# ChampiB/CBO_with_OOP

Measured on AMD Instinct MI355X. Metric: candidate-intervention acquisitions/sec (16k grid, d=3), higher is better.
Workload: dtype f64

## Files before the change

cbo_with_oop_amd/csrc/kernels_trsm.hip:

```cpp
#include <cstdlib>
#include <type_traits>

#include "cbo_internal.h"

namespace cbo {

#define MFMA_F64(a, b, c) __builtin_amdgcn_mfma_f64_16x16x4f64((a), (b), (c), 0, 0, 0)

#define SCHED_DS(n) __builtin_amdgcn_sched_group_barrier(0x100, (n), 0)
#define SCHED_MFMA(n) __builtin_amdgcn_sched_group_barrier(0x008, (n), 0)
#define SCHED_VMEM(n) __builtin_amdgcn_sched_group_barrier(0x010, (n), 0)

constexpr int kRB = 128;
constexpr int kT = kRB / 16;
constexpr int kLdsLd = kRB + 16;
constexpr int kNBuf = 3;
template <int KB>
struct StageGeom {
    static constexpr int kA = KB * kLdsLd;
    static constexpr int kB = 4 * KB * 16;
    static constexpr int kRA = KB / 4;
    static constexpr int kParts = KB / 8;
    static constexpr int kDma = 3 * kParts;
    static constexpr int kKS = KB / 4;
// ... 950 lines not shown
                    }
                    x = MFMA_F64(iv[2], -acc[m][2], x);
                    x2 = MFMA_F64(iv[3], -acc[m][3], x2);
                    __builtin_amdgcn_sched_barrier(0);
                    x += x2;
                    asm volatile("" : "+v"(x));
#pragma unroll
                    for (int r = 0; r < 4; ++r) xreg[(kq + 4 * r) * 16 + lc] = x[r];
                    PSTAMP(3);
                    asm volatile("s_waitcnt lgkmcnt(0)" ::: "memory");
                    __builtin_amdgcn_s_barrier();
                    __builtin_amdgcn_s_setprio(0);
                    PSTAMP(1);
#pragma unroll
                    for (int t = m + 1; t < kT; ++t)
#pragma unroll
                        for (int kk = 0; kk < 4; ++kk) uf[t][kk] = abase0[(4 * kk) * kPLd + 16 * t];
                    if (SWEEP) {
#pragma unroll
                        for (int r = 0; r < 4; ++r) zr[r] = zl[zpar + 16 * m + kq + 4 * r];
                    }
#pragma unroll
                    for (int kk = 0; kk < 4; ++kk) {
                        if (m + 1 < kT) acc[m + 1] = MFMA_F64(uf[m + 1][kk], x[kk], acc[m + 1]);
                        if (m + 2 < kT) acc[m + 2] = MFMA_F64(uf[m + 2][kk], x[kk], acc[m + 2]);
                        __builtin_amdgcn_sched_barrier(0);
                        if (kk == 0) { issue_one(ahead, bnext, 0); issue_one(ahead, bnext, 1); }
                        else if (kk == 1) { issue_one(ahead, bnext, 2); issue_one(ahead, bnext, 3); }
                        else if (kk == 2) issue_one(ahead, bnext, 4);
                        else advance(ahead);
                        __builtin_amdgcn_sched_barrier(0);
                    }
#pragma unroll
                    for (int r = 0; r < 4; ++r) {
                        asm volatile("global_store_dwordx2 %0, %1, %2" ::"v"(vq_off), "v"(x[r]), "s"(V + colw + (int64_t)(i0 + 16 * m + 4 * r) * ldv) : "memory");
                        if (SWEEP) {
                            qacc = fma(x[r], x[r], qacc);
                            macc = fma(x[r], zr[r], macc);
                        }
                    }
                    if (SWEEP) asm volatile("" : "+v"(qacc), "+v"(macc));
#pragma unroll
                    for (int kk = 0; kk < 4; ++kk)
#pragma unroll
                        for (int t = m + 3; t < kT; ++t) acc[t] = MFMA_F64(uf[t][kk], x[kk], acc[t]);
                    a1 += 4;
                    if (SWEEP && m == kPD0 - 1) {
                        hand[0] = qacc;
                        hand[1] = macc;
                        qacc = 0.0;
                        macc = 0.0;
                    }
                    PSTAMP(2); PSTAMP_NEXT(); buf = (buf == 2) ? 0 : buf + 1;
                }
#pragma unroll
                for (int m = 0; m < kPD1; ++m) {
                    wait_top();
                    const int bnext = (buf >= 1) ? buf - 1 : 2;
                    issue_stage(ahead, bnext);
                    advance(ahead);
                    if (m < 2) {
#pragma unroll
                        for (int sl = (m == 0 ? 0 : kL0); sl < (m == 0 ? kL0 : kAhead); ++sl) {
                            request_one(i0, sl);
                            __builtin_amdgcn_s_sleep(2);
                        }
                        a1 += m == 0 ? kL0 : kL1;
                    }
                    PSTAMP(2); PSTAMP_NEXT(); buf = (buf == 2) ? 0 : buf + 1;
                }
            } else {
#pragma unroll
                for (int m = 0; m < kPD0; ++m) {
                    wait_top();
                    const int bnext = (buf >= 1) ? buf - 1 : 2;
                    const double *abase0 = lds + buf * kPA + kq * kPLd + lc;
                    double *xreg = ldsB + buf * kPBd + cw * 256;
                    double uf[kT][4], xb[4];
#pragma unroll
                    for (int t = 0; t < kT; ++t) {
                        if (m > 0 || !P0) acc[t] = MFMA_F64(af[1][t], bf[1], acc[t]);
#pragma unroll
                        for (int kk = 0; kk < 4; ++kk) uf[t][kk] = abase0[(4 * kk) * kPLd + kRB + 16 * t];
                    }
                    PSTAMP(3);
                    asm volatile("s_waitcnt lgkmcnt(0)" ::: "memory");
                    __builtin_amdgcn_s_barrier();
                    PSTAMP(1);
#pragma unroll
                    for (int kk = 0; kk < 4; ++kk) xb[kk] = xreg[(4 * kk + kq) * 16 + lc];
#pragma unroll
                    for (int kk = 0; kk < (m + 1 < kPD0 ? 3 : 4); ++kk)
#pragma unroll
                        for (int t = 0; t < kT; ++t) {
                            acc[t] = MFMA_F64(uf[t][kk], xb[kk], acc[t]);
                            const int slot = kk * kT + t;
                            if (slot < kPDma) issue_one(ahead, bnext, slot);
                            else if (slot == kPDma) step(ahead);
                            else if (slot == kPDma + 1) locate_a(ahead);
                            else if (slot == kPDma + 2) locate_b(ahead);
                            else if (slot == kPDma + 3) locate_c(ahead);
                            __builtin_amdgcn_sched_barrier(0);
                        }
                    if (m + 1 < kPD0) {
#pragma unroll
                        for (int t = 0; t < kT; ++t) af[1][t] = uf[t][3];
                        bf[1] = xb[3];
                    }
                    PSTAMP(2); PSTAMP_NEXT(); buf = (buf == 2) ? 0 : buf + 1;
                }
#pragma unroll
                for (int m = 0; m < kPD1; ++m) {
                    wait_top();
                    const int bnext = (buf >= 1) ? buf - 1 : 2;
                    constexpr int kTl = kT;
                    const int s = 2 * m;
                    const double *ab = lds + buf * kPA + kq * kPLd + lc;
                    const double *ivb = ldsB + buf * kPBd + kq * 16 + lc;
                    double iv[2][4], uf[2][kTl][4], zr[2][4];
                    if (SWEEP && m == 0) {
                        qacc = hand[0];
                        macc = hand[1];
                    }
#pragma unroll
                    for (int kk = 0; kk < 4; ++kk) iv[0][kk] = ivb[(4 * kk) * 16];
                    d4 x = {0.0, 0.0, 0.0, 0.0}, x2 = {0.0, 0.0, 0.0, 0.0};
                    x = MFMA_F64(iv[0][0], -acc[s][0], x);
                    x2 = MFMA_F64(iv[0][1], -acc[s][1], x2);
                    x = MFMA_F64(iv[0][2], -acc[s][2], x);
                    x2 = MFMA_F64(iv[0][3], -acc[s][3], x2);
                    __builtin_amdgcn_sched_barrier(0);
#pragma unroll
                    for (int kk = 0; kk < 4; ++kk) iv[1][kk] = ivb[256 + (4 * kk) * 16];
#pragma unroll
                    for (int t = s + 1; t < kT; ++t)
#pragma unroll
                        for (int kk = 0; kk < 4; ++kk) uf[0][t][kk] = ab[(4 * kk) * kPLd + 16 * t];
                    if (SWEEP) {
#pragma unroll
                        for (int hh = 0; hh < 2; ++hh)
#pragma unroll
                            for (int r = 0; r < 4; ++r) zr[hh][r] = zl[zpar + kRB + 16 * (s + hh) + kq + 4 * r];
                    }
                    __builtin_amdgcn_sched_barrier(0);
                    x += x2;
                    asm volatile("" : "+v"(x));
                    PSTAMP(1);
                    auto emit = [&](int hh, const d4 &xx) __attribute__((always_inline)) {
#pragma unroll
                        for (int r = 0; r < 4; ++r) {
                            asm volatile("global_store_dwordx2 %0, %1, %2" ::"v"(vq_off), "v"(xx[r]), "s"(V + colw + (int64_t)(i0 + kRB + 16 * (s + hh) + 4 * r) * ldv) : "memory");
                            if (SWEEP) {
                                qacc = fma(xx[r], xx[r], qacc);
                                macc = fma(xx[r], zr[hh][r], macc);
                            }
                        }
                        if (SWEEP) asm volatile("" : "+v"(qacc), "+v"(macc));
                    };
#pragma unroll
                    for (int kk = 0; kk < 4; ++kk) {
                        acc[s + 1] = MFMA_F64(uf[0][s + 1][kk], x[kk], acc[s + 1]);
                        if (s + 2 < kT) acc[s + 2] = MFMA_F64(uf[0][s + 2][kk], x[kk], acc[s + 2]);
                        __builtin_amdgcn_sched_barrier(0);
                        if (kk == 0) { issue_one(ahead, bnext, 0); issue_one(ahead, bnext, 1); }
                        else if (kk == 1) { issue_one(ahead, bnext, 2); issue_one(ahead, bnext, 3); }
                        else if (kk == 2) issue_one(ahead, bnext, 4);
                        else advance(ahead);
                        __builtin_amdgcn_sched_barrier(0);
                    }
                    emit(0, x);
                    const d4 na = -acc[s + 1];
                    d4 y1 = {0.0, 0.0, 0.0, 0.0}, y2 = {0.0, 0.0, 0.0, 0.0};
#pragma unroll
                    for (int kk = 0; kk < 4; ++kk) {
                        if (kk & 1) y2 = MFMA_F64(iv[1][kk], na[kk], y2);
                        else y1 = MFMA_F64(iv[1][kk], na[kk], y1);
#pragma unroll
                        for (int t = s + 3; t < kT; ++t) {
                            acc[t] = MFMA_F64(uf[0][t][kk], x[kk], acc[t]);
                            if (SWEEP && m == 1 && kk == 0 && t == s + 3) request_one(i0, kT * 4);
                        }
                    }
#pragma unroll
                    for (int t = s + 2; t < kT; ++t)
#pragma unroll
                        for (int kk = 0; kk < 4; ++kk) uf[1][t][kk] = ab[(4 * kk) * kPLd + kRB + 16 * t];
                    const d4 y = y1 + y2;
                    emit(1, y);
#pragma unroll
                    for (int kk = 0; kk < 4; ++kk)
#pragma unroll
                        for (int t = s + 2; t < kT; ++t) {
                            acc[t] = MFMA_F64(uf[1][t][kk], y[kk], acc[t]);
                            const int idx = kk * (kT - s - 2) + (t - s - 2);
                            if (m < 2 && idx < 16) request_one(i0, 16 * m + idx);
                        }
                    a1 += 8 + (m == 0 ? kL0 : m == 1 ? kL1 : 0);
                    if (SWEEP && m == kPD1 - 1) {
                        qacc += __shfl_xor(qacc, 16);
                        qacc += __shfl_xor(qacc, 32);
                        macc += __shfl_xor(macc, 16);
                        macc += __shfl_xor(macc, 32);
                        qtot += qacc;
                        mtot += macc;
                        qacc = 0.0;
                        macc = 0.0;
                    }
                    PSTAMP(2); PSTAMP_NEXT(); buf = (buf == 2) ? 0 : buf + 1;
                }
            }
        };
        diag_phase(0, std::true_type{});
        for (int i0 = kPB; i0 < n; i0 += kPB) {
            const int nst = i0 / kPKB;
            regular_stage(i0, std::true_type{});
            for (int j = 1; j < nst; ++j) regular_stage(i0, std::false_type{});
            diag_phase(i0, std::false_type{});
        }
        asm volatile("s_waitcnt vmcnt(0)" ::: "memory");
        __builtin_amdgcn_s_barrier();

        if (SWEEP && H == 1 && kq == 0) {
            q_out[colw + lc] = qtot;
            mu_out[colw + lc] = mtot;
        }
    };
    if (h == 0) run(std::integral_constant<int, 0>{});
    else run(std::integral_constant<int, 1>{});
#undef PSTAMP
#undef PSTAMP_NEXT
}

constexpr int kAccMoves = kT * 4;

template <int KB>
__global__ __launch_bounds__(256) void trsm_update_kernel(const double *__restrict__ U, int64_t ldu,
                                                          const double *V, int64_t ldv, double *C, int64_t ldc, int k0,
                                                          int klen, int i0_begin, int i0_end, int chunk_rows,
                                                          int upper_only, const int *__restrict__ skip_if)
{
    if (skip_if && __builtin_nontemporal_load(skip_if) != 0) return;
    using G = StageGeom<KB>;
    constexpr int kA = G::kA, kB = G::kB, kRA = G::kRA, kParts = G::kParts, kDma = G::kDma, kKS = G::kKS;
    __shared__ __align__(16) double lds[kNBuf * (kA + kB)];

    const int tid = threadIdx.x;
#ifdef CBO_DIAG_KNOBS
    const unsigned long long upd_t0 = __builtin_amdgcn_s_memtime();
    const unsigned long long upd_r0 = __builtin_amdgcn_s_memrealtime();
    const int upd_id = (int)(blockIdx.y * gridDim.x + blockIdx.x);
    const bool upd_probe = tid == 0 && blockIdx.x == 7 && blockIdx.y == gridDim.y / 2;
    int upd_k = 0;
#define UPD_STAMP() do { if (upd_probe && upd_k < 128) g_upd_stage[upd_k++] = __builtin_amdgcn_s_memtime(); } while (0)
#else
#define UPD_STAMP() do { } while (0)
#endif
    const int lane = tid & 63;
    const int wave = __builtin_amdgcn_readfirstlane(tid >> 6);
    const int lc = lane & 15, kq = lane >> 4;
    const int64_t colw = (int64_t)blockIdx.x * kStrip + wave * 16;
    const int ib = i0_begin + (int)blockIdx.y * chunk_rows;
    const int ie = (ib + chunk_rows < i0_end) ? ib + chunk_rows : i0_end;
    if (ib >= ie) return;
    if (upper_only && (int)blockIdx.x * kStrip + kStrip <= ib) return;
    const int nst = klen / KB;
    double *Cc = C + colw + lc;
    double *ldsB = lds + kNBuf * kA;
    const unsigned lds_byte0 = lds_byte_address(lds);
    const double *ug = U + (int64_t)(k0 + wave * kRA) * ldu + lane * 2;
    const double *vg = V + (int64_t)(k0 + (lane >> 3)) * ldv + colw + 2 * (lane & 7);
    const int64_t b_stride = 8 * ldv;

    int ci0 = ib, cj = 0;
    const double *a_src, *b_src;
    auto locate = [&]() __attribute__((always_inline)) {
        const bool past = ci0 >= ie;
        const int ai0 = past ? ie - kRB : ci0;
        const int aj = past ? nst - 1 : cj;
        a_src = ug + (int64_t)(KB * aj) * ldu + ai0;
        b_src = vg + (int64_t)(KB * aj) * ldv;
    };
    auto advance = [&]() __attribute__((always_inline)) {
        const int wrap = (cj + 1 == nst) ? 1 : 0;
        ci0 += kRB * wrap;
        cj = (cj + 1) * (1 - wrap);
        locate();
    };
    auto issue_one = [&](int buf, int part, int q) __attribute__((always_inline)) {
        if (q < 2) {
            const unsigned la = __builtin_amdgcn_readfirstlane(lds_byte0 + 8u * (unsigned)(buf * kA + (wave * kRA) * kLdsLd));
            const int p = 2 * part + q;
            glds16(a_src + (int64_t)p * ldu, la + 8u * (unsigned)(p * kLdsLd));
        } else {
            const unsigned lb = __builtin_amdgcn_readfirstlane(
                lds_byte0 + 8u * (unsigned)(kNBuf * kA + buf * kB + wave * (KB * 16)));
            glds16(b_src + part * b_stride, lb + 8u * (unsigned)(part * 128));
        }
    };
    auto issue_part = [&](int buf, int part) __attribute__((always_inline)) {
#pragma unroll
        for (int q = 0; q < 3; ++q) issue_one(buf, part, q);
    };

    d4 acc[kT], accn[kT];
#pragma unroll
    for (int t = 0; t < kT; ++t)
#pragma unroll
        for (int r = 0; r < 4; ++r) acc[t][r] = -Cc[(int64_t)(ib + 16 * t + kq + 4 * r) * ldc];

    UPD_STAMP();
    locate();
#pragma unroll
    for (int part = 0; part < kParts; ++part) issue_part(0, part);
    advance();
#pragma unroll
    for (int part = 0; part < kParts; ++part) issue_part(1, part);
    advance();
    UPD_STAMP();

    int buf = 0;
    int boundary = 0;
    for (int i0 = ib; i0 < ie; i0 += kRB) {
        double af[2][kT], bf[2];
        bool deferred = false;
        for (int j = 0; j < nst; ++j) {
            asm volatile("s_waitcnt lgkmcnt(0)" ::: "memory");
            if (boundary) asm volatile("s_waitcnt vmcnt(%0)" ::"n"(kDma + kAccMoves) : "memory");
            else asm volatile("s_waitcnt vmcnt(%0)" ::"n"(kDma) : "memory");
            __builtin_amdgcn_s_barrier();
            UPD_STAMP();
            boundary = (boundary > 0) ? boundary - 1 : 0;
            if (j == 0 && i0 + kRB < ie) {
#pragma unroll
                for (int t = 0; t < kT; ++t)
#pragma unroll
                    for (int r = 0; r < 4; ++r) accn[t][r] = -Cc[(int64_t)(i0 + kRB + 16 * t + kq + 4 * r) * ldc];
                asm volatile("" ::: "memory");
            }
            __builtin_amdgcn_sched_barrier(0);
            const int bnext = (buf >= 1) ? buf - 1 : 2;
            const double *abase = lds + buf * kA + kq * kLdsLd + lc;
            const double *bbase = ldsB + buf * kB + wave * (KB * 16) + kq * 16 + lc;
#pragma unroll
            for (int t = 0; t < kT; ++t) {
                if (deferred) acc[t] = MFMA_F64(af[1][t], bf[1], acc[t]);
                if (t < kT / 2) {
                    af[0][2 * t] = abase[32 * t];
                    af[0][2 * t + 1] = abase[32 * t + 16];
                } else if (t == kT / 2) {
                    bf[0] = bbase[0];
                }
                __builtin_amdgcn_sched_barrier(0);
            }
#pragma unroll
            for (int jj = 0; jj < kKS - 1; ++jj) {
                const double *an = abase + 4 * (jj + 1) * kLdsLd;
#pragma unroll
                for (int t = 0; t < kT; ++t) {
                    acc[t] = MFMA_F64(af[jj & 1][t], bf[jj & 1], acc[t]);
                    if (t < kT / 2) {
                        af[(jj + 1) & 1][2 * t] = an[32 * t];
                        af[(jj + 1) & 1][2 * t + 1] = an[32 * t + 16];
                    } else if (t == kT / 2) {
                        bf[(jj + 1) & 1] = bbase[4 * (jj + 1) * 16];
                    } else if (jj < kParts) {
                        issue_one(bnext, jj, t - (kT / 2 + 1));
                    } else if (jj == kParts && t == kT / 2 + 1) {
                        advance();
                    }
                    __builtin_amdgcn_sched_barrier(0);
                }
            }
            deferred = true;
            buf = (buf == 2) ? 0 : buf + 1;
        }
#pragma unroll
        for (int t = 0; t < kT; ++t) acc[t] = MFMA_F64(af[1][t], bf[1], acc[t]);
        UPD_STAMP();
#pragma unroll
        for (int t = 0; t < kT; ++t)
#pragma unroll
            for (int r = 0; r < 4; ++r) Cc[(int64_t)(i0 + 16 * t + kq + 4 * r) * ldc] = -acc[t][r];
        asm volatile("" ::: "memory");
        UPD_STAMP();
#pragma unroll
        for (int t = 0; t < kT; ++t) acc[t] = accn[t];
        boundary = 2;
    }
    asm volatile("s_waitcnt vmcnt(0)" ::: "memory");
    __builtin_amdgcn_s_barrier();
#ifdef CBO_DIAG_KNOBS
    UPD_STAMP();
    if (tid == 0 && upd_id < 65536) {
        unsigned hw, xcc;
        asm volatile("s_getreg_b32 %0, hwreg(HW_REG_HW_ID)" : "=s"(hw));
        asm volatile("s_getreg_b32 %0, hwreg(HW_REG_XCC_ID)" : "=s"(xcc));
        g_upd_wg[5 * upd_id] = upd_t0;
        g_upd_wg[5 * upd_id + 1] = __builtin_amdgcn_s_memtime();
        g_upd_wg[5 * upd_id + 2] = (unsigned long long)hw | ((unsigned long long)xcc << 32);
        g_upd_wg[5 * upd_id + 3] = upd_r0;
        g_upd_wg[5 * upd_id + 4] = __builtin_amdgcn_s_memrealtime();
    }
#endif
#undef UPD_STAMP
}

void launch_trsm_strips(hipStream_t s, const double *U, int64_t ldu, const double *invDt, double *V, int64_t ldv,
                        int64_t n, int64_t m_pad, const double *z, double *q, double *mu, bool accumulate,
                        bool half_lds)
{
    if (n <= 0 || m_pad <= 0) return;
    const dim3 grid((unsigned)(m_pad / kStrip));
    const int acc = accumulate ? 1 : 0;
    if (half_lds) {
        if (q != nullptr)
            hipLaunchKernelGGL((trsm_strip_kernel<true, 16>), grid, dim3(256), 0, s, U, ldu, invDt, V, ldv, (int)n, z, q, mu, acc);
        else
            hipLaunchKernelGGL((trsm_strip_kernel<false, 16>), grid, dim3(256), 0, s, U, ldu, invDt, V, ldv, (int)n, z, q, mu, 0);
        return;
    }
    static const bool pairs = [] {
        const char *e = getenv("CBO_HIP_STRIP_FORM");
        return !(e && atoi(e) == 8);
    }();
    if (pairs && n >= kPB && n % kPB == 0) {
#ifdef CBO_DIAG_KNOBS
        static const int pair_mask = [] {
            const char *e = getenv("CBO_HIP_STRIP_MASK");
            return e ? atoi(e) : 0;
        }();
        const int acc = (accumulate ? 1 : 0) | (pair_mask << 8);
#endif
        if (q != nullptr)
            hipLaunchKernelGGL((trsm_pair_kernel<true>), grid, dim3(512), 0, s, U, ldu, invDt, V, ldv, (int)n, z, q, mu, acc);
        else
            hipLaunchKernelGGL((trsm_pair_kernel<false>), grid, dim3(512), 0, s, U, ldu, invDt, V, ldv, (int)n, z, q, mu, 0);
        return;
    }
    if (q != nullptr)
        hipLaunchKernelGGL((trsm_strip8_kernel<true>), grid, dim3(512), 0, s, U, ldu, invDt, V, ldv, (int)n, z, q, mu, acc);
    else
        hipLaunchKernelGGL((trsm_strip8_kernel<false>), grid, dim3(512), 0, s, U, ldu, invDt, V, ldv, (int)n, z, q, mu, 0);
}

void launch_trsm_update(hipStream_t s, const double *U, int64_t ldu, double *V, int64_t ldv, int k0, int klen,
                        int i0_begin, int i0_end, int64_t m_pad, int chunk_blocks, bool half_lds)
{
    launch_gemm_update(s, U, ldu, V, ldv, V, ldv, k0, klen, i0_begin, i0_end, m_pad, chunk_blocks, half_lds, false, nullptr);
}

void launch_gemm_update(hipStream_t s, const double *U, int64_t ldu, const double *V, int64_t ldv, double *C,
                        int64_t ldc, int k0, int klen, int i0_begin, int i0_end, int64_t m_pad, int chunk_blocks,
                        bool half_lds, bool upper_only, const int *skip_if)
{
    if (i0_begin >= i0_end || m_pad <= 0 || klen <= 0) return;
    const int chunk_rows = chunk_blocks * kRB;
    const unsigned chunks = (unsigned)((i0_end - i0_begin + chunk_rows - 1) / chunk_rows);
    const dim3 grid((unsigned)(m_pad / kStrip), chunks);
    const int up = upper_only ? 1 : 0;
    if (!half_lds)
        hipLaunchKernelGGL(trsm_update_kernel<32>, grid, dim3(256), 0, s, U, ldu, V, ldv, C, ldc, k0, klen, i0_begin,
                           i0_end, chunk_rows, up, skip_if);
    else
        hipLaunchKernelGGL(trsm_update_kernel<16>, grid, dim3(256), 0, s, U, ldu, V, ldv, C, ldc, k0, klen, i0_begin,
                           i0_end, chunk_rows, up, skip_if);
}

__global__ void mfma_selftest_kernel(const double *A, const double *B, double *C)
{
    const int l = threadIdx.x;
    d4 acc = {0.0, 0.0, 0.0, 0.0};
    for (int k0 = 0; k0 < 16; k0 += 4)
        acc = MFMA_F64(A[(l & 15) * 16 + k0 + (l >> 4)], B[(k0 + (l >> 4)) * 16 + (l & 15)], acc);
    d4 acc2 = {0.0, 0.0, 0.0, 0.0};
    for (int kk = 0; kk < 4; ++kk) acc2 = MFMA_F64(A[(l & 15) * 16 + 4 * kk + (l >> 4)], acc[kk], acc2);
    for (int r = 0; r < 4; ++r) {
        C[((l >> 4) + 4 * r) * 16 + (l & 15)] = acc[r];
        C[256 + ((l >> 4) + 4 * r) * 16 + (l & 15)] = acc2[r];
    }
}

int run_mfma_selftest(hipStream_t s, double *max_err)
{
    double hA[256], hB[256], hC[512], ref[256], ref2[256];
    for (int i = 0; i < 16; ++i)
        for (int j = 0; j < 16; ++j) {
            hA[i * 16 + j] = (double)((i * 7 + j * 3) % 11 - 5);
            hB[i * 16 + j] = (double)((i * 5 + j * 13 + 1) % 17 - 8);
        }
    for (int i = 0; i < 16; ++i)
        for (int j = 0; j < 16; ++j) {
            double acc = 0.0;
            for (int k = 0; k < 16; ++k) acc += hA[i * 16 + k] * hB[k * 16 + j];
            ref[i * 16 + j] = acc;
        }
    for (int i = 0; i < 16; ++i)
        for (int j = 0; j < 16; ++j) {
            double acc = 0.0;
            for (int k = 0; k < 16; ++k) acc += hA[i * 16 + k] * ref[k * 16 + j];
            ref2[i * 16 + j] = acc;
        }
    double *dA = nullptr, *dB = nullptr, *dC = nullptr;
    if (hipMalloc(&dA, sizeof(hA)) != hipSuccess || hipMalloc(&dB, sizeof(hB)) != hipSuccess ||
        hipMalloc(&dC, sizeof(hC)) != hipSuccess)
        return -1;
    hipMemcpyAsync(dA, hA, sizeof(hA), hipMemcpyHostToDevice, s);
    hipMemcpyAsync(dB, hB, sizeof(hB), hipMemcpyHostToDevice, s);
    hipLaunchKernelGGL(mfma_selftest_kernel, dim3(1), dim3(64), 0, s, dA, dB, dC);
    hipMemcpyAsync(hC, dC, sizeof(hC), hipMemcpyDeviceToHost, s);
    const hipError_t e = hipStreamSynchronize(s);
    hipFree(dA); hipFree(dB); hipFree(dC);
    if (e != hipSuccess) return -1;
    double m = 0.0;
    for (int i = 0; i < 256; ++i) {
        const double e1 = fabs(hC[i] - ref[i]), e2 = fabs(hC[256 + i] - ref2[i]);
        if (e1 > m) m = e1;
        if (e2 > m) m = e2;
    }
    *max_err = m;
    return 0;
}

}
```

Before: 3.053 million.

## Prefetch next C strip via inline-asm loads spread across stages with tracked vmcnt

Replaces the compiler-generated prefetch of the next accumulator strip, which was issued in one burst at stage 0, with inline-asm global loads. These are split into two batches of 16, issued after the MFMA loops of stages 0 and 1. A young-load counter selects the matching s_waitcnt vmcnt so the LDS DMA waits do not also wait on the C prefetch. The negation of the loaded C values moves until after the initial DMA issue or the strip boundary. This is meant to hide C load latency behind MFMA work and avoid stalls at strip boundaries. In exchange it relies on fragile manual vmcnt accounting (including kAccMoves) and carries a correctness risk if the counts mismatch.

```diff
diff --git a/cbo_with_oop_amd/csrc/kernels_trsm.hip b/cbo_with_oop_amd/csrc/kernels_trsm.hip
--- a/cbo_with_oop_amd/csrc/kernels_trsm.hip
+++ b/cbo_with_oop_amd/csrc/kernels_trsm.hip
@@ -1276,13 +1276,13 @@
         for (int q = 0; q < 3; ++q) issue_one(buf, part, q);
     };
 
-    d4 acc[kT], accn[kT];
+    d4 acc[kT];
+    double accn[kT][4];
 #pragma unroll
     for (int t = 0; t < kT; ++t)
 #pragma unroll
-        for (int r = 0; r < 4; ++r) acc[t][r] = -Cc[(int64_t)(ib + 16 * t + kq + 4 * r) * ldc];
-
-    UPD_STAMP();
+        for (int r = 0; r < 4; ++r) acc[t][r] = Cc[(int64_t)(ib + 16 * t + kq + 4 * r) * ldc];
+
     locate();
 #pragma unroll
     for (int part = 0; part < kParts; ++part) issue_part(0, part);
@@ -1291,26 +1291,33 @@
     for (int part = 0; part < kParts; ++part) issue_part(1, part);
     advance();
     UPD_STAMP();
+    __builtin_amdgcn_sched_barrier(0);
+#pragma unroll
+    for (int t = 0; t < kT; ++t) acc[t] = -acc[t];
+    UPD_STAMP();
 
     int buf = 0;
-    int boundary = 0;
+    const unsigned c_off = (unsigned)(((int64_t)kq * ldc + lc) * 8);
+    auto request_one = [&](int i0, int sl) __attribute__((always_inline)) {
+        const double *cb = C + colw + (int64_t)(i0 + kRB + 16 * (sl >> 2) + 4 * (sl & 3)) * ldc;
+        asm volatile("global_load_dwordx2 %0, %1, %2" : "=v"(accn[sl >> 2][sl & 3]) : "v"(c_off), "s"(cb) : "memory");
+    };
+    int young1 = 0, young2 = 0;
     for (int i0 = ib; i0 < ie; i0 += kRB) {
         double af[2][kT], bf[2];
         bool deferred = false;
+        const bool ahead = i0 + kRB < ie;
         for (int j = 0; j < nst; ++j) {
             asm volatile("s_waitcnt lgkmcnt(0)" ::: "memory");
-            if (boundary) asm volatile("s_waitcnt vmcnt(%0)" ::"n"(kDma + kAccMoves) : "memory");
-            else asm volatile("s_waitcnt vmcnt(%0)" ::"n"(kDma) : "memory");
+            const int young = young1 + young2;
+            if (young == 0) asm volatile("s_waitcnt vmcnt(%0)" ::"n"(kDma) : "memory");
+            else if (young == 16) asm volatile("s_waitcnt vmcnt(%0)" ::"n"(kDma + 16) : "memory");
+            else if (young == 32) asm volatile("s_waitcnt vmcnt(%0)" ::"n"(kDma + 32) : "memory");
+            else asm volatile("s_waitcnt vmcnt(%0)" ::"n"(kDma + 48) : "memory");
             __builtin_amdgcn_s_barrier();
             UPD_STAMP();
-            boundary = (boundary > 0) ? boundary - 1 : 0;
-            if (j == 0 && i0 + kRB < ie) {
-#pragma unroll
-                for (int t = 0; t < kT; ++t)
-#pragma unroll
-                    for (int r = 0; r < 4; ++r) accn[t][r] = -Cc[(int64_t)(i0 + kRB + 16 * t + kq + 4 * r) * ldc];
-                asm volatile("" ::: "memory");
-            }
+            young2 = young1;
+            young1 = 0;
             __builtin_amdgcn_sched_barrier(0);
             const int bnext = (buf >= 1) ? buf - 1 : 2;
             const double *abase = lds + buf * kA + kq * kLdsLd + lc;
@@ -1345,6 +1352,17 @@
                     __builtin_amdgcn_sched_barrier(0);
                 }
             }
+            if (j < 2 && ahead) {
+                if (j == 0) {
+#pragma unroll
+                    for (int sl = 0; sl < 16; ++sl) request_one(i0, sl);
+                } else {
+#pragma unroll
+                    for (int sl = 16; sl < 32; ++sl) request_one(i0, sl);
+                }
+                young1 = 16;
+            }
+            __builtin_amdgcn_sched_barrier(0);
             deferred = true;
             buf = (buf == 2) ? 0 : buf + 1;
         }
@@ -1357,11 +1375,17 @@
             for (int r = 0; r < 4; ++r) Cc[(int64_t)(i0 + 16 * t + kq + 4 * r) * ldc] = -acc[t][r];
         asm volatile("" ::: "memory");
         UPD_STAMP();
-#pragma unroll
-        for (int t = 0; t < kT; ++t) acc[t] = accn[t];
-        boundary = 2;
+        asm volatile("s_waitcnt vmcnt(%0)" ::"n"(kDma + kAccMoves) : "memory");
+#pragma unroll
+        for (int t = 0; t < kT; ++t)
+#pragma unroll
+            for (int r = 0; r < 4; ++r) {
+                asm volatile("; ahead-pin %0" : "+v"(accn[t][r]));
+                acc[t][r] = -accn[t][r];
+            }
+        young1 += kAccMoves;
     }
-    asm volatile("s_waitcnt vmcnt(0)" ::: "memory");
+    asm volatile("s_waitcnt vmcnt(%0)" ::"n"(kAccMoves) : "memory");
     __builtin_amdgcn_s_barrier();
 #ifdef CBO_DIAG_KNOBS
     UPD_STAMP();
```

Result: no change. 3.034 million (median of 6 runs) (-0.6%).
